# kei312/stereoanywhere

Hardware: AMD Instinct MI355X
Metric: stereo pairs/sec @540x960 D=192 (1/2/4/8 GPU) + EPE vs reference (higher is better)
Workload: dtype f32 (F(4x4) Winograd-domain and direct-conv products as exact f16 hi/lo pair products on MFMA, fp32 accumulation; everything else fp32); 1 GPU; configs[1]: batch 4/GPU x 540x960 (padded 544x960), 22 GRU iters, published flags; global_batch=4, iters=22, parallelism=dp1 (independent pairs, metrics all_gather)

## Files before the change

stereoanywhere_amd/csrc/conv2d_wino4.hip:

```cpp
#include "sa_common.h"

#include <algorithm>
#include <cstdlib>
#include <type_traits>

#pragma clang fp contract(fast)

namespace {

using sa::f32x4, sa::f32x2, sa::f16x2, sa::f16x4;

constexpr int NPT = 36;

template <int NW_, int KC_, bool SPLIT_ = false>
struct W4Cfg {
  static constexpr bool SPLIT = SPLIT_;
  static constexpr int NW = NW_, NTHR = 64 * NW_, TG = NW_ / 2, NT = 16 * TG, KC = KC_, JPC = KC_ / 4;
  static constexpr int NR = 6;
  static constexpr int CO = 32, CG = 2;
  static constexpr int SB = 4 * CO;
  static constexpr int PS_MAX = NT == 64 ? 340 : 204;
  static constexpr int PBUF = (KC * PS_MAX + 63) / 64 * 64 * 4;
  static constexpr int UBUF = NPT * KC * CO;
  static constexpr int BUF = PBUF + UBUF;
  static constexpr int OPP = NT * 16 + 4;
  static constexpr int SMEM = 2 * BUF > CO * OPP + CO * 9 + 8 ? 2 * BUF : CO * OPP + CO * 9 + 8;
  static constexpr int PDMA = ((KC * PS_MAX + 63) / 64 + NW - 1) / NW;
  static constexpr int UDMA = UBUF / 256;
  static constexpr int UPW = (UDMA + NW - 1) / NW;
  static_assert(SMEM * 4 <= 160 * 1024, "LDS budget");
  static constexpr int PPART = (PDMA > UPW ? PDMA : UPW) > 6 ? 3 : 2;
  static_assert(PDMA <= 3 * PPART && UPW <= 3 * PPART, "three DMA parts");
  static_assert(OPP % 32 == 4, "conflict-free staging");
  static constexpr int AFF_MAX = (160 * 1024 - SMEM * 4) / 8 > 512 ? 512 : (160 * 1024 - SMEM * 4) / 8;
};
using W4Big = W4Cfg<8, 8>;
using W4Small = W4Cfg<4, 4>;
using W4Split = W4Cfg<8, 8, true>;
constexpr int W4S_LOG2 = 12;
struct W4Half : W4Cfg<8, 8, true> {
  static constexpr bool HALF = true;
};
template <class C, class = void>
struct W4IsHalf : std::false_type {};
template <class C>
struct W4IsHalf<C, std::enable_if_t<C::HALF>> : std::true_type {};
static_assert(2 * W4Small::SMEM * 4 <= 160 * 1024, "two small blocks per CU");
template <class C, bool AFF>
constexpr bool W4Paired = C::SPLIT && C::JPC == 2 && !(W4IsHalf<C>::value && AFF);
constexpr int W4_GJB = 4;
constexpr int W4_GJB1 = 8;

struct W4Prob {
  const float *in;
  long in_bs;
  int Cin, H, W;
  const float *U;
  int Cout;
  const float *bias;
  int relu;
  float *out;
  long out_bs;
  int ltw;
  int tiles_w, tiles_hw, co_blocks;
  double *partial;
  const float *in_m, *in_s, *in_t;
  int in_pstride, in_act;
  int pitch;
  const float *skip;
  long skip_bs;
  const float *skip_s, *skip_t;
  int skip_act, out_act;
};
constexpr int MAX_PROB = 8;

__device__ __forceinline__ void w4_item(const unsigned wid, const int co_blocks, const int tiles_hw, int &cb, int &st,
                                        int &n) {
  cb = wid % co_blocks;
  const int gt = wid / co_blocks;
  st = gt % tiles_hw;
  n = gt / tiles_hw;
}
struct W4Gate {
  int mode;
  const float *ctx;
  long ctx_bs;
  const float *h;
  long h_bs;
  const float *z;
  long z_bs;
  const float *add;
  long add_bs;
  float *out2;
  long out2_bs;
  const float *head_w;
  float *head_part;
  long head_part_bs;
};
struct W4Launch {
  W4Prob p[MAX_PROB];
  W4Gate gate[MAX_PROB];
  unsigned end[MAX_PROB];
  unsigned nblk[MAX_PROB];
  int nprob;
  int guard;
};

__device__ __forceinline__ void w4_pair_split(const float x0, const float x1, f16x4 &ahi, f16x4 &alo) {
  const f16x2 h0 = __builtin_convertvector(f32x2{x0, x0}, f16x2);
  const f16x2 h1 = __builtin_convertvector(f32x2{x1, x1}, f16x2);
  float l0, l1;
  asm("v_fma_mix_f32 %0, -%1, 1.0, %2 op_sel_hi:[1,0,0]" : "=v"(l0) : "v"(__builtin_bit_cast(unsigned, h0)), "v"(x0));
  asm("v_fma_mix_f32 %0, -%1, 1.0, %2 op_sel_hi:[1,0,0]" : "=v"(l1) : "v"(__builtin_bit_cast(unsigned, h1)), "v"(x1));
  const f16x2 q0 = __builtin_convertvector(f32x2{l0, 0.0f}, f16x2);
  const f16x2 q1 = __builtin_convertvector(f32x2{l1, 0.0f}, f16x2);
  ahi = __builtin_shufflevector(h0, h1, 0, 1, 2, 3);
  alo = __builtin_shufflevector(q0, q1, 0, 1, 2, 3);
}

__device__ __forceinline__ f16x4 w4_pair_half(const float x0, const float x1) {
  const f16x2 h0 = __builtin_convertvector(f32x2{x0, x0}, f16x2);
  const f16x2 h1 = __builtin_convertvector(f32x2{x1, x1}, f16x2);
  return __builtin_shufflevector(h0, h1, 0, 1, 2, 3);
}

__device__ unsigned g_w4_redo_blocks;

__device__ __forceinline__ void dma16(__amdgpu_buffer_rsrc_t r, float *lds, int voff, int soff) {
  __builtin_amdgcn_raw_ptr_buffer_load_lds(r, (__attribute__((address_space(3))) void *)lds, 16, voff, soff, 0, 0);
}

__device__ __forceinline__ void bt6(const float x0, const float x1, const float x2, const float x3, const float x4,
                                    const float x5, float *o) {
  const float a = fmaf(-4.0f, x2, x4), b = fmaf(-4.0f, x1, x3), c = x4 - x2, e = x3 - x1;
  o[0] = fmaf(4.0f, x0, fmaf(-5.0f, x2, x4));
  o[1] = a + b;
  o[2] = a - b;
  o[3] = fmaf(2.0f, e, c);
  o[4] = fmaf(-2.0f, e, c);
  o[5] = fmaf(4.0f, x1, fmaf(-5.0f, x3, x5));
}

__device__ __forceinline__ void at6(const float *m, float *o) {
  const float a = m[1] + m[2], b = m[1] - m[2], c = m[3] + m[4], e = m[3] - m[4];
  o[0] = m[0] + a + c;
  o[1] = b + 2.0f * e;
  o[2] = a + 4.0f * c;
  o[3] = b + 8.0f * e + m[5];
}

template <int H>
__device__ __forceinline__ f32x4 at6h(const float u0, const float u1, const float u2) {
  if (H == 0) {
    const float p = u1 + u2, q = u1 - u2;
    return f32x4{u0 + p, q, p, q};
  } else {
    const float p = u0 + u1, q = u0 - u1;
    return f32x4{p, 2.0f * q, 4.0f * p, 8.0f * q + u2};
  }
}

__device__ __forceinline__ int w4_tile_of_row(int m) {
  const bool mid = m >= 4 && m < 12;
  const int j = mid ? m - 4 : (m < 4 ? m : m - 8);
  return (mid ? 0 : 2) + 4 * (j >> 1) + (j & 1);
}

template <int HF>
__device__ __forceinline__ void bt6h(const float x0, const float x1, const float x2, const float x3, const float x4,
                                     const float x5, float *o) {
  if (HF == 0) {
    const float a = fmaf(-4.0f, x2, x4), b = fmaf(-4.0f, x1, x3);
    o[0] = fmaf(4.0f, x0, fmaf(-5.0f, x2, x4));
    o[1] = a + b;
    o[2] = a - b;
  } else {
    const float c = x4 - x2, e = x3 - x1;
    o[0] = fmaf(2.0f, e, c);
    o[1] = fmaf(-2.0f, e, c);
    o[2] = fmaf(4.0f, x1, fmaf(-5.0f, x3, x5));
  }
}

template <class C, bool GATED, int NCH>
__device__ __forceinline__ void w4_emit(const W4Prob &P, const W4Gate *gate, const float *ot, const int cbase,
                                        const int n, const int co0, const int st, const int tiles_w, const int y0,
                                        const int x0, const int BH, const int BW, const int lbw, const int tid) {
  constexpr int NT = C::NT, NTHR = C::NTHR, OPP = C::OPP;
  const int H = P.H, W = P.W, Cout = P.Cout, pitch = P.pitch, hw = H * pitch;
  const int cb0 = co0 + cbase;
  auto tail0 = [&](f32x4 v, const int x) __attribute__((always_inline)) {
    if (x + 4 > W) {
#pragma unroll
      for (int e = 0; e < 4; ++e)
        if (x + e >= W) v[e] = 0.0f;
    }
    return v;
  };
  if (P.partial) {
    constexpr int NSUB = NT / 32, TPC = NTHR / (NCH * NSUB), PPT = 32 * 16 / TPC;
    const int c = tid / (TPC * NSUB), sub = (tid / TPC) % NSUB, part = tid % TPC;
    const int sub_rows = BH / NSUB, fine_h = (H + sub_rows - 1) / sub_rows;
    const int frow = (st / tiles_w) * NSUB + sub;
    double ssum = 0.0, ssq = 0.0;
#pragma unroll 2
    for (int p = sub * 512 + part * PPT; p < sub * 512 + (part + 1) * PPT; p += 4) {
      const int r = p >> lbw, cx = p & (BW - 1);
      if (y0 + r < H && x0 + cx < W) {
        const f32x4 v = tail0(*reinterpret_cast<const f32x4 *>(ot + c * OPP + p), x0 + cx);
#pragma unroll
        for (int e = 0; e < 4; ++e) {
          const double d = v[e];
          ssum += d;
          ssq += d * d;
        }
      }
    }
#pragma unroll
    for (int o = TPC / 2; o > 0; o >>= 1) {
      ssum += __shfl_xor(ssum, o);
      ssq += __shfl_xor(ssq, o);
    }
    if (part == 0 && frow < fine_h) {
      const long fst = (long)frow * tiles_w + st % tiles_w;
      double *pp = P.partial + (((long)n * Cout + cb0 + c) * ((long)fine_h * tiles_w) + fst) * 2;
      pp[0] = ssum;
      pp[1] = ssq;
    }
  }
  float *dst = P.out + (long)n * P.out_bs;
  constexpr int NJ = (NCH * NT * 16) / (4 * NTHR);
  auto plain_stores = [&]() __attribute__((always_inline)) {
    if (P.skip) {
      const float *sk = P.skip + (long)n * P.skip_bs;
#pragma unroll 4
      for (int j = 0; j < NJ; ++j) {
        const int i4 = tid + NTHR * j;
        const int c = i4 / (NT * 4), p = (i4 % (NT * 4)) * 4, r = p >> lbw, cx = p & (BW - 1);
        const int y = y0 + r, x = x0 + cx;
        if (y < H && x < W) {
          const long off = (long)(cb0 + c) * hw + (long)y * pitch + x;
          const f32x4 sv = *reinterpret_cast<const f32x4 *>(sk + off);
          const float ss = P.skip_s ? P.skip_s[cb0 + c] : 1.0f, st_ = P.skip_t ? P.skip_t[cb0 + c] : 0.0f;
          f32x4 v = *reinterpret_cast<const f32x4 *>(ot + c * OPP + p);
#pragma unroll
          for (int e = 0; e < 4; ++e) {
            float a = sv[e] * ss + st_;
            if (P.skip_act) a = fmaxf(a, 0.0f);
            v[e] = v[e] + a;
            if (P.out_act) v[e] = fmaxf(v[e], 0.0f);
          }
          *reinterpret_cast<f32x4 *>(dst + off) = tail0(v, x);
        }
      }
      return;
    }
#pragma unroll 4
    for (int j = 0; j < NJ; ++j) {
      const int i4 = tid + NTHR * j;
      const int c = i4 / (NT * 4), p = (i4 % (NT * 4)) * 4, r = p >> lbw, cx = p & (BW - 1);
      const int y = y0 + r, x = x0 + cx;
      if (y < H && x < W)
        *reinterpret_cast<f32x4 *>(dst + (long)(cb0 + c) * hw + (long)y * pitch + x) =
            tail0(*reinterpret_cast<const f32x4 *>(ot + c * OPP + p), x);
    }
  };
  if constexpr (!GATED) {
    plain_stores();
    return;
  } else {
  const W4Gate &GT = *gate;
  if (GT.mode == 0) {
    plain_stores();
    return;
  }
  const int half = Cout / 2;
// ... 123 lines not shown

template <class C, int LTW>
struct W4Geo {
  static constexpr int tw = 1 << LTW, tr = C::NT >> LTW;
  static constexpr int BH = 4 * tr, BW = 4 * tw, PG = tw + 2, PR = BH + 2, PS = PR * PG;
};

template <class C, bool AFF>
__device__ __forceinline__ float w4_guard_scale(const W4Prob &P, float *smem, const int n, const int nchunks,
                                                const int hw, const int (&po)[C::PDMA], const unsigned pcs,
                                                const int wv, const int lane) {
  constexpr int NWAVE = C::NW, KC = C::KC, PDMA = C::PDMA;
  float *red = smem;
  const char *ib = reinterpret_cast<const char *>(P.in + (long)n * P.in_bs);
  float mx = 0.0f;
#pragma unroll 8
  for (int kc = 0; kc < nchunks; ++kc)
#pragma unroll
    for (int j = 0; j < PDMA; ++j) {
      const int pcj = (int)((pcs >> (4 * j)) & 15u) - 1;
      if (pcj < 0) continue;
      const f32x4 v = *reinterpret_cast<const f32x4 *>(ib + po[j] + (long)kc * KC * hw * 4);
      float a = 1.0f, b = 0.0f, fl = -INFINITY;
      if constexpr (AFF) {
        const int pi = n * P.in_pstride + kc * KC + pcj;
        const float m0 = P.in_m ? P.in_m[pi] : 0.0f, t0 = P.in_t ? P.in_t[pi] : 0.0f;
        a = P.in_s ? P.in_s[pi] : 1.0f;
        b = t0 - m0 * a;
        fl = P.in_act ? 0.0f : -INFINITY;
      }
#pragma unroll
      for (int e = 0; e < 4; ++e) {
        const float t = __builtin_fabsf(fmaxf(v[e] * a + b, fl));
        mx = fmaxf(mx, t < INFINITY ? t : 0.0f);
      }
    }
  mx = sa::wave_max_dpp(mx);
  if (lane == 0) red[wv] = mx;
  __syncthreads();
  mx = red[0];
#pragma unroll
  for (int w = 1; w < NWAVE; ++w) mx = fmaxf(mx, red[w]);
  __syncthreads();
  int e2;
  (void)frexpf(100.0f * mx, &e2);
  return mx > 0.0f ? ldexpf(1.0f, 15 - e2) : 1.0f;
}

template <class C, int HF, int LTW, bool GATED, bool AFF>
__device__ __forceinline__ bool w4_body(const W4Prob &P, const W4Gate *gate, const unsigned wid, float *smem,
                                        float2 *atab, const bool guard = false, float xscale = 1.0f) {
  constexpr int NWAVE = C::NW, NTHR = C::NTHR, KC = C::KC, JPC = C::JPC, PDMA = C::PDMA,
                UDMA = C::UDMA, UPW = C::UPW, UBUF = C::UBUF, BUF = C::BUF, PBUF = C::PBUF, OPP = C::OPP,
                CO = C::CO, CG = C::CG, SB = C::SB, NR = C::NR;
  constexpr bool SPLIT = C::SPLIT, HALF = W4IsHalf<C>::value;
  static_assert(!SPLIT || NWAVE == 8, "split: the 8-wave shape");
  using f32xg = float __attribute__((ext_vector_type(CG)));
  const int Cin = P.Cin, H = P.H;
  using Geo = W4Geo<C, LTW>;
  constexpr int ltw = LTW, tw = Geo::tw, BH = Geo::BH, BW = Geo::BW, PG = Geo::PG, PS = Geo::PS;
  const int tid = threadIdx.x;
  const int lane = tid & 63;
  const int wv = __builtin_amdgcn_readfirstlane(tid >> 6);
  const int co_blocks = P.co_blocks, tiles_hw = P.tiles_hw, tiles_w = P.tiles_w;
  int cb, st, n;
  w4_item(wid, co_blocks, tiles_hw, cb, st, n);
  const int y0 = (st / tiles_w) * BH, x0 = (st % tiles_w) * BW;
  const int co0 = cb * CO;
  const int pitch = P.pitch, hw = H * pitch;
  const int nchunks = Cin / KC;

  const __amdgpu_buffer_rsrc_t xin = __builtin_amdgcn_make_buffer_rsrc(
      const_cast<float *>(P.in + (long)n * P.in_bs), (short)0, Cin * hw * 4, 0x00020000);
  const __amdgpu_buffer_rsrc_t uin = __builtin_amdgcn_make_buffer_rsrc(
      const_cast<float *>(P.U + (long)cb * Cin * NPT * CO), (short)0, Cin * NPT * CO * 4, 0x00020000);
  auto u_src = [&](int piece) {
    const int f = piece * 256 + lane * 4;
    return (JPC == 2 ? f : f + (f / SB) * SB) * 4;
  };
  auto u_chunk = [&](int chunk) {
    return JPC == 2 ? chunk * UBUF * 4 : (chunk >> 1) * 2 * UBUF * 4 + (chunk & 1) * SB * 4;
  };

#pragma unroll
  for (int j = 0; j < UPW; ++j)
    if (wv + NWAVE * j < UDMA)
      dma16(uin, smem + PBUF + (wv + NWAVE * j) * 256, u_src(wv + NWAVE * j), u_chunk(0));
  const int npi = (KC * PS + 63) >> 6;
  int po[PDMA];
  unsigned pcs = 0;
  static_assert(PDMA <= 8 && KC < 15, "4-bit channel fields");
#pragma unroll
  for (int j = 0; j < PDMA; ++j) {
    const int s = (wv + NWAVE * j) * 64 + lane;
    const int ci = s / PS, rem = s - ci * PS, r = rem / PG, g = rem - r * PG;
    const int y = y0 - 1 + r, x = x0 - 4 + 4 * g;
    const bool ok = s < KC * PS && y >= 0 && y < H && x >= 0 && x < pitch;
    po[j] = ok ? (ci * hw + y * pitch + x) * 4 : 0x7ffffff0;
    pcs |= (ok && wv + NWAVE * j < (KC * PS + 63) / 64 ? (unsigned)ci + 1u : 0u) << (4 * j);
  }
  if constexpr (SPLIT) {
    if (xscale == 0.0f) xscale = w4_guard_scale<C, AFF>(P, smem, n, nchunks, hw, po, pcs, wv, lane);
  }
  const bool scaled = xscale != 1.0f;
  auto issue_part = [&](int chunk, int buf, int part) __attribute__((always_inline)) {
    float *pb = smem + buf * BUF;
    const int xs = chunk * KC * hw * 4;
    float *ub = pb + PBUF;
    const int us = u_chunk(chunk);
#pragma unroll
    for (int j = 0; j < PDMA; ++j)
      if ((part < 0 || j / C::PPART == part) && wv + NWAVE * j < npi) dma16(xin, pb + (wv + NWAVE * j) * 256, po[j], xs);
#pragma unroll
    for (int j = 0; j < UPW; ++j)
      if ((part < 0 || j / C::PPART == part) && wv + NWAVE * j < UDMA)
        dma16(uin, ub + (wv + NWAVE * j) * 256, u_src(wv + NWAVE * j), us);
  };
  auto issue_p0 = [&]() __attribute__((always_inline)) {
#pragma unroll
    for (int j = 0; j < PDMA; ++j)
      if (wv + NWAVE * j < npi) dma16(xin, smem + (wv + NWAVE * j) * 256, po[j], 0);
  };

  const int tg = wv % C::TG;
  const int k = lane >> 4, m = lane & 15;
  const int tidx = tg * 16 + w4_tile_of_row(m), trow = tidx >> ltw, tcol = tidx & (tw - 1);
  int PSv = PS, PGv = PG;
  asm volatile("" : "+s"(PSv), "+s"(PGv));
  const int pread = k * PSv * 4 + 4 * trow * PGv * 4 + 4 * tcol + 2;
  const int uread = (k * 16 + m) * CG * (SPLIT ? JPC : 1);

  f32x4 acc[NR][3][CG];
#pragma unroll
  for (int i = 0; i < NR; ++i)
#pragma unroll
    for (int jj = 0; jj < 3; ++jj)
#pragma unroll
      for (int g = 0; g < CG; ++g) acc[i][jj][g] = f32x4{0.f, 0.f, 0.f, 0.f};

  float bpre[CG / 2];
#pragma unroll
  for (int k = 0; k < CG / 2; ++k) bpre[k] = P.bias ? P.bias[co0 + (2 * k + HF) * 16 + (lane & 15)] : 0.0f;
  if (HF == 1) __builtin_amdgcn_s_setprio(1);
  issue_p0();
  const float act_floor = P.in_act ? 0.0f : -INFINITY;
  if constexpr (AFF) {
    for (int c = tid; c < Cin; c += NTHR) {
      const int pi = n * P.in_pstride + c;
      const float m0 = P.in_m ? P.in_m[pi] : 0.0f, sc = P.in_s ? P.in_s[pi] : 1.0f, t0 = P.in_t ? P.in_t[pi] : 0.0f;
      atab[c] = make_float2(sc * xscale, (t0 - m0 * sc) * xscale);
    }
    __syncthreads();
  }
#pragma unroll 1
  for (int kc = 0; kc < nchunks; ++kc) {
    const int cur = kc & 1;
    if constexpr (AFF) {
      asm volatile("s_waitcnt vmcnt(0)" ::: "memory");
      float *pbuf = smem + cur * BUF;
#pragma unroll
      for (int j = 0; j < PDMA; ++j) {
        const int pcj = (int)((pcs >> (4 * j)) & 15u) - 1;
        if (pcj >= 0) {
          f32x4 *q = reinterpret_cast<f32x4 *>(pbuf + ((wv + NWAVE * j) * 64 + lane) * 4);
          const float2 ab = atab[kc * KC + pcj];
          f32x4 v = *q;
#pragma unroll
          for (int e = 0; e < 4; ++e) v[e] = fmaxf(v[e] * ab.x + ab.y, act_floor);
          *q = v;
        }
      }
    }
    if constexpr (SPLIT && !AFF) {
      if (scaled) {
        asm volatile("s_waitcnt vmcnt(0)" ::: "memory");
        float *pbuf = smem + cur * BUF + (wv * 64 + lane) * 4;
#pragma unroll 1
        for (int j = 0; j < PDMA; ++j) {
          if (wv + NWAVE * j < npi) {
            f32x4 *q = reinterpret_cast<f32x4 *>(pbuf + NWAVE * j * 256);
            *q = *q * xscale;
          }
        }
      }
    }
    __syncthreads();
    const float *pb = smem + cur * BUF + pread;
    const float *ub = smem + cur * BUF + PBUF + uread;
    f32x2 ra[6], rc[6];
    f32x4 rb[6];
    auto load_rows = [&](int s, int r0, int r1) __attribute__((always_inline)) {
      const float *p = pb + s * 4 * PSv * 4;
#pragma unroll
      for (int r = r0; r < r1; ++r) {
        ra[r] = *reinterpret_cast<const f32x2 *>(p + r * PGv * 4);
        rb[r] = *reinterpret_cast<const f32x4 *>(p + r * PGv * 4 + 2);
        rc[r] = *reinterpret_cast<const f32x2 *>(p + r * PGv * 4 + 6);
      }
    };
    f32xg bc[NR], bn[NR];
    auto load_b = [&](int s, int jj, f32xg *b) __attribute__((always_inline)) {
#pragma unroll
      for (int i = 0; i < NR; ++i) {
        if constexpr (SPLIT) {
          const float *q = ub + (6 * i + 3 * HF + jj) * JPC * SB + s;
          b[i] = f32xg{q[0], q[JPC]};
        } else {
          b[i] = *reinterpret_cast<const f32xg *>(ub + ((6 * i + 3 * HF + jj) * JPC + s) * SB);
        }
      }
    };
    if constexpr (W4Paired<C, AFF>) {
      float t0[6][3], t1[6][3];
      load_rows(0, 0, 6);
#pragma unroll
      for (int r = 0; r < 6; ++r) bt6h<HF>(ra[r].y, rb[r].x, rb[r].y, rb[r].z, rb[r].w, rc[r].x, t0[r]);
      load_rows(1, 0, 6);
#pragma unroll
      for (int r = 0; r < 6; ++r) bt6h<HF>(ra[r].y, rb[r].x, rb[r].y, rb[r].z, rb[r].w, rc[r].x, t1[r]);
      f32x4 pc_[NR];
      auto load_bp = [&](int jj, int i0, int i1, f32x4 (&b)[NR]) __attribute__((always_inline)) {
#pragma unroll
        for (int i = i0; i < i1; ++i) b[i] = *reinterpret_cast<const f32x4 *>(ub + (6 * i + 3 * HF + jj) * JPC * SB);
      };
#pragma unroll
      for (int jj = 0; jj < 3; ++jj) {
        if (kc + 1 < nchunks) {
          issue_part(kc + 1, cur ^ 1, jj);
          __builtin_amdgcn_sched_barrier(0);
        }
        load_bp(jj, 0, NR / 2, pc_);
        float v0[6], v1[6];
        bt6(t0[0][jj], t0[1][jj], t0[2][jj], t0[3][jj], t0[4][jj], t0[5][jj], v0);
        bt6(t1[0][jj], t1[1][jj], t1[2][jj], t1[3][jj], t1[4][jj], t1[5][jj], v1);
#pragma unroll
        for (int i = 0; i < NR; ++i) {
          if (i == 1) load_bp(jj, NR / 2, NR, pc_);
          if constexpr (HALF) {
            const f16x4 ahi = w4_pair_half(v0[i], v1[i]);
#pragma unroll
            for (int g = 0; g < CG; ++g) {
              const f16x4 bp = __builtin_bit_cast(f16x4, g == 0 ? pc_[i].xy : pc_[i].zw);
              acc[i][jj][g] = __builtin_amdgcn_mfma_f32_16x16x16f16(ahi, bp, acc[i][jj][g], 0, 0, 0);
            }
          } else {
            f16x4 ahi, alo;
            w4_pair_split(v0[i], v1[i], ahi, alo);
#pragma unroll
            for (int g = 0; g < CG; ++g) {
              const f16x4 bp = __builtin_bit_cast(f16x4, g == 0 ? pc_[i].xy : pc_[i].zw);
              acc[i][jj][g] = __builtin_amdgcn_mfma_f32_16x16x16f16(ahi, bp, acc[i][jj][g], 0, 0, 0);
              acc[i][jj][g] = __builtin_amdgcn_mfma_f32_16x16x16f16(alo, bp, acc[i][jj][g], 0, 0, 0);
            }
          }
        }
        __builtin_amdgcn_sched_barrier(0);
      }
    } else {
      load_rows(0, 0, 6);
      load_b(0, 0, bc);
#pragma unroll
      for (int s = 0; s < JPC; ++s) {
        if (s == 1) load_rows(1, 3, 6);
        float t[6][3];
#pragma unroll
        for (int r = 0; r < 6; ++r) bt6h<HF>(ra[r].y, rb[r].x, rb[r].y, rb[r].z, rb[r].w, rc[r].x, t[r]);
        if (s + 1 < JPC) load_rows(1, 0, 3);
#pragma unroll
        for (int jj = 0; jj < 3; ++jj) {
          if (s == 0 && kc + 1 < nchunks) {
            issue_part(kc + 1, cur ^ 1, jj);
            __builtin_amdgcn_sched_barrier(0);
          }
          if (s + 1 < JPC || jj < 2) load_b(jj < 2 ? s : s + 1, jj < 2 ? jj + 1 : 0, bn);
          float v[6];
          bt6(t[0][jj], t[1][jj], t[2][jj], t[3][jj], t[4][jj], t[5][jj], v);
          if constexpr (SPLIT) {
            static_assert(HALF, "an unpaired split config is the half config");
#pragma unroll
            for (int i = 0; i < NR; ++i) {
              const f16x4 a = __builtin_shufflevector(__builtin_convertvector(f32x2{v[i], v[i]}, f16x2),
                                                      f16x2{(_Float16)0.0f, (_Float16)0.0f}, 0, 1, 2, 3);
              const f16x4 b0 = __builtin_bit_cast(f16x4, f32x2{bc[i][0], bc[i][0]});
              const f16x4 b1 = __builtin_bit_cast(f16x4, f32x2{bc[i][1], bc[i][1]});
              acc[i][jj][0] = __builtin_amdgcn_mfma_f32_16x16x16f16(a, b0, acc[i][jj][0], 0, 0, 0);
              acc[i][jj][1] = __builtin_amdgcn_mfma_f32_16x16x16f16(a, b1, acc[i][jj][1], 0, 0, 0);
            }
          } else {
#pragma unroll
            for (int i = 0; i < NR; ++i)
#pragma unroll
              for (int g = 0; g < CG; ++g)
                acc[i][jj][g] = __builtin_amdgcn_mfma_f32_16x16x4f32(v[i], bc[i][g],
                                                                      acc[i][jj][g], 0, 0, 0);
          }
          __builtin_amdgcn_sched_barrier(0);

#pragma unroll
          for (int i = 0; i < NR; ++i) bc[i] = bn[i];
        }
      }
    }
  }
  __syncthreads();
  if constexpr (SPLIT) {
    const float inv_scale = 1.0f / ((float)(1 << W4S_LOG2) * xscale);
#pragma unroll
    for (int i = 0; i < NR; ++i)
#pragma unroll
      for (int jj = 0; jj < 3; ++jj)
#pragma unroll
        for (int g = 0; g < CG; ++g) acc[i][jj][g] *= inv_scale;
  }

  float *ot = smem;
  const int relu = P.relu;
  f32x4 chk = f32x4{0.f, 0.f, 0.f, 0.f};
  float whead = 0.0f;
  if constexpr (GATED && C::NTHR == 512)
    if (gate->mode == 3 && tid < C::CO * 9) whead = gate->head_w[co0 * 9 + tid];
#pragma unroll
  for (int phase = 0; phase < 2; ++phase) {
#pragma unroll
  for (int gi = 0; gi < CG / 2; ++gi) {
    const int g = 2 * gi + (phase == 0 ? 1 - HF : HF);
    const int col = g * 16 + (lane & 15);
    const float bv = phase == 1 ? bpre[gi] : 0.0f;
#pragma unroll
    for (int i = 0; i < 4; ++i) {
      const int ti = tg * 16 + w4_tile_of_row(4 * (lane >> 4) + i), orow = (ti >> ltw) * 4, ocol = (ti & (tw - 1)) * 4;
      float u[4][3];
#pragma unroll
      for (int jj = 0; jj < 3; ++jj) {
        float mcol[6], o[4];
#pragma unroll
        for (int a = 0; a < 6; ++a) mcol[a] = acc[a][jj][g][i];
        at6(mcol, o);
#pragma unroll
        for (int a = 0; a < 4; ++a) u[a][jj] = o[a];
      }
#pragma unroll
      for (int a = 0; a < 4; ++a) {
        const f32x4 y = at6h<HF>(u[a][0], u[a][1], u[a][2]);
        f32x4 *o = reinterpret_cast<f32x4 *>(ot + col * OPP + (orow + a) * BW + ocol);
        if (phase == 0) {
          *o = y;
        } else {
          f32x4 v = (HF == 0 ? (*o + y) : (y + *o)) + bv;
          if constexpr (SPLIT) chk += v;
          if (relu) v = f32x4{fmaxf(v.x, 0.0f), fmaxf(v.y, 0.0f), fmaxf(v.z, 0.0f), fmaxf(v.w, 0.0f)};
          *o = v;
        }
      }
    }
  }
    if (phase == 0) __syncthreads();
  }
  if constexpr (SPLIT) {
    static_assert(C::CO * C::OPP + C::CO * 9 + NWAVE <= C::SMEM, "range guard flags");
    int *flags = reinterpret_cast<int *>(smem + C::CO * C::OPP + C::CO * 9);
    const float t = (chk.x + chk.y) + (chk.z + chk.w);
    const bool wbad = __builtin_amdgcn_ballot_w64(!__builtin_isfinite(t)) != 0;
    if (lane == 0) flags[wv] = wbad ? 1 : 0;
    __syncthreads();
    int any = 0;
#pragma unroll
    for (int w = 0; w < NWAVE; ++w) any |= flags[w];
    if (any && guard) return true;
  } else {
    __syncthreads();
  }
  if constexpr (GATED && C::NTHR == 512) {
    if (gate->mode == 3) {
      w4_flowhead<C, LTW>(P, *gate, smem, n, co0, st, y0, x0, tid, whead);
      return false;
    }
  }
  w4_emit<C, GATED, C::CO>(P, gate, ot, 0, n, co0, st, tiles_w, y0, x0, BH, BW, ltw + 2, tid);
  return false;
}

template <class C, bool GATED, bool AFF = false>
__global__ __launch_bounds__(C::NTHR, C::NW == 8 ? 1 : 2) void wino_f4k3_kernel(const W4Launch L) {
  const unsigned g = blockIdx.x;
  int pi = 0;
#pragma unroll
  for (int i = 1; i < MAX_PROB; ++i) pi += (i < L.nprob && g >= L.end[i - 1]) ? 1 : 0;
  const unsigned base = pi ? L.end[pi - 1] : 0u, nb = L.nblk[pi];
  if (g - base >= nb) return;
  __shared__ __attribute__((aligned(16))) float smem[C::SMEM];
  __shared__ float2 atab[AFF ? C::AFF_MAX : 1];
  const unsigned wid = sa::xcd_remap(g - base, nb);
  const bool guard = C::SPLIT && L.guard;
  const W4Prob &P = L.p[pi];
  const W4Gate *gp = GATED ? &L.gate[pi] : nullptr;
  bool over;
#define W4_BODY(CC_, HF_, LTW_, G_, XS_) w4_body<CC_, HF_, LTW_, GATED, AFF>(P, gp, wid, smem, atab, G_, XS_)
  if (threadIdx.x < C::NTHR / 2) over = P.ltw == 4 ? W4_BODY(C, 0, 4, guard, 1.0f) : W4_BODY(C, 0, 5, guard, 1.0f);
  else over = P.ltw == 4 ? W4_BODY(C, 1, 4, guard, 1.0f) : W4_BODY(C, 1, 5, guard, 1.0f);
  if constexpr (C::SPLIT) {
    if (over) {
      __syncthreads();
      if (threadIdx.x == 0) atomicAdd(&g_w4_redo_blocks, 1u);
      int pil = __builtin_amdgcn_readfirstlane(pi);
      unsigned widl = __builtin_amdgcn_readfirstlane(wid);
      asm volatile("" : "+s"(pil), "+s"(widl));
      const W4Prob &P2 = L.p[pil];
      const W4Gate *gp2 = GATED ? &L.gate[pil] : nullptr;
#define W4_BODY2(HF_, LTW_) w4_body<C, HF_, LTW_, GATED, AFF>(P2, gp2, widl, smem, atab, false, 0.0f)
      if (threadIdx.x < C::NTHR / 2) {
        if (P2.ltw == 4) W4_BODY2(0, 4);
        else W4_BODY2(0, 5);
      } else {
        if (P2.ltw == 4) W4_BODY2(1, 4);
        else W4_BODY2(1, 5);
      }
#undef W4_BODY2
    }
  }
#undef W4_BODY
}

__global__ __launch_bounds__(256) void wino4_weights_kernel(const float *__restrict__ w, int Cout, int Cin, int CB,
                                                            float *__restrict__ U) {
  const long i = (long)blockIdx.x * blockDim.x + threadIdx.x;
  if (i >= (long)Cout * Cin) return;
  const int co = (int)(i / Cin), ci = (int)(i % Cin);
  const float *g = w + i * 9;
  const double G[6][3] = {{0.25, 0.0, 0.0},
                          {-1.0 / 6, -1.0 / 6, -1.0 / 6},
                          {-1.0 / 6, 1.0 / 6, -1.0 / 6},
                          {1.0 / 24, 1.0 / 12, 1.0 / 6},
                          {1.0 / 24, -1.0 / 12, 1.0 / 6},
                          {0.0, 0.0, 1.0}};
  double t[6][3];
  for (int a = 0; a < 6; ++a)
    for (int c = 0; c < 3; ++c) t[a][c] = G[a][0] * g[c] + G[a][1] * g[3 + c] + G[a][2] * g[6 + c];
  const int chunk = ci / 8, s = (ci % 8) / 4, k = ci % 4, cb = co / CB, c = co % CB, ng = CB / 16;
  for (int a = 0; a < 6; ++a)
    for (int b = 0; b < 6; ++b) {
      const double u = t[a][0] * G[b][0] + t[a][1] * G[b][1] + t[a][2] * G[b][2];
      const int pt = 6 * a + b;
      U[(((((long)cb * (Cin / 8) + chunk) * NPT + pt) * 2 + s) * 4 + k) * CB + (c & 15) * ng + (c >> 4)] = (float)u;
    }
}

__global__ __launch_bounds__(256) void wino4s_weights_kernel(const float *__restrict__ w, int Cout, int Cin,
                                                             unsigned *__restrict__ U) {
  const long i = (long)blockIdx.x * blockDim.x + threadIdx.x;
  if (i >= (long)Cout * Cin) return;
  const int co = (int)(i / Cin), ci = (int)(i % Cin);
  const float *g = w + i * 9;
  const double G[6][3] = {{0.25, 0.0, 0.0},
                          {-1.0 / 6, -1.0 / 6, -1.0 / 6},
                          {-1.0 / 6, 1.0 / 6, -1.0 / 6},
                          {1.0 / 24, 1.0 / 12, 1.0 / 6},
                          {1.0 / 24, -1.0 / 12, 1.0 / 6},
                          {0.0, 0.0, 1.0}};
  double t[6][3];
  for (int a = 0; a < 6; ++a)
    for (int c = 0; c < 3; ++c) t[a][c] = G[a][0] * g[c] + G[a][1] * g[3 + c] + G[a][2] * g[6 + c];
  const int chunk = ci / 8, s = (ci % 8) / 4, k = ci % 4, cb = co / 32, gg = (co % 32) / 16, n = co % 16;
  for (int a = 0; a < 6; ++a)
    for (int b = 0; b < 6; ++b) {
      const double u = (t[a][0] * G[b][0] + t[a][1] * G[b][1] + t[a][2] * G[b][2]) * (double)(1 << W4S_LOG2);
      const _Float16 hi = (_Float16)(float)u;
      const _Float16 lo = (_Float16)(float)(u - (double)hi);
      const unsigned pr = (unsigned)__builtin_bit_cast(unsigned short, hi) |
                          ((unsigned)__builtin_bit_cast(unsigned short, lo) << 16);
      const int pt = 6 * a + b;
      U[((((((long)cb * (Cin / 8) + chunk) * NPT + pt) * 4 + k) * 16 + n) * 2 + gg) * 2 + s] = pr;
    }
}


__global__ __launch_bounds__(256) void flow_head_reduce_kernel(const float *__restrict__ part, long part_bs, int ncb,
                                                               int H, int W, int BH, int BW, int tiles_w,
                                                               int tiles_hw, const float *__restrict__ bias0,
                                                               float *__restrict__ cx, float *__restrict__ fa,
                                                               long fa_bs, float *__restrict__ fb, long fb_bs) {
  const unsigned r = blockIdx.x * 256u + threadIdx.x;
  const unsigned hw = (unsigned)(H * W);
  if (r >= hw) return;
  const long b = blockIdx.y;
  const int y = (int)(r / (unsigned)W), x = (int)(r % (unsigned)W);
  const int RH = BH + 2, RW = BW + 2, tiles_h = tiles_hw / tiles_w;
  const int ty0 = y / BH, tx0 = x / BW;
  const bool up = y % BH == 0 && ty0 > 0, dn = y % BH == BH - 1 && ty0 + 1 < tiles_h;
  const bool lf = x % BW == 0 && tx0 > 0, rt = x % BW == BW - 1 && tx0 + 1 < tiles_w;
  const int ty1 = up ? ty0 - 1 : ty0 + 1, tx1 = lf ? tx0 - 1 : tx0 + 1;
  auto off = [&](int ty, int tx) { return ((long)(ty * tiles_w + tx) * RH + (y - (ty * BH - 1))) * RW + (x - (tx * BW - 1)); };
  const bool hy = up || dn, hx = lf || rt;
  const long o0 = off(ty0, tx0), o1 = hx ? off(ty0, tx1) : o0, o2 = hy ? off(ty1, tx0) : o0,
             o3 = hx && hy ? off(ty1, tx1) : o0;
  float d = bias0[0];
  const float *pc = part + b * part_bs;
  const long cbs = (long)tiles_hw * RH * RW;
  for (int cb0 = 0; cb0 < ncb; cb0 += 8) {
    float a[8][4];
#pragma unroll
    for (int j = 0; j < 8; ++j) {
      const float *q = pc + (long)min(cb0 + j, ncb - 1) * cbs;
      a[j][0] = q[o0];
      a[j][1] = q[o1];
      a[j][2] = q[o2];
      a[j][3] = q[o3];
    }
#pragma unroll
    for (int j = 0; j < 8; ++j) {
      const bool in = cb0 + j < ncb;
      d = in ? d + a[j][0] : d;
      d = in && hx ? d + a[j][1] : d;
      d = in && hy ? d + a[j][2] : d;
      d = in && hx && hy ? d + a[j][3] : d;
    }
  }
  const long i = b * hw + r;
  const float c = cx[i] + d;
  cx[i] = c;
  const float fx = c - (float)x;
  if (fa) {
    fa[b * fa_bs + r] = fx;
    fa[b * fa_bs + hw + r] = 0.0f;
  }
  if (fb) {
    fb[b * fb_bs + r] = fx;
    fb[b * fb_bs + hw + r] = 0.0f;
  }
}

int w4_ltw(int H, int W) {
  const long a16 = (long)((W + 63) / 64) * 64 * ((H + 15) / 16) * 16;
  const long a32 = (long)((W + 127) / 128) * 128 * ((H + 7) / 8) * 8;
  return a32 < a16 ? 5 : 4;
}

}

extern "C" int sa_conv2d_wino4_weights(const float *weight, int Cout, int Cin, float *U, void *stream) {
  SA_REQUIRE(weight && U && Cout > 0 && Cin > 0 && Cin % 8 == 0 && Cout % 32 == 0,
             "sa_conv2d_wino4_weights: bad arguments (Cin %% 8, Cout %% 32)");
  const long n = (long)Cout * Cin;
  hipStream_t s = sa::as_stream(stream);
  wino4_weights_kernel<<<(unsigned)((n + 255) / 256), 256, 0, s>>>(weight, Cout, Cin, 32, U);
  return sa::check_launch("sa_conv2d_wino4_weights");
}

extern "C" int sa_conv2d_wino4_weights_split(const float *weight, int Cout, int Cin, void *U, void *stream) {
  SA_REQUIRE(weight && U && Cout > 0 && Cin > 0 && Cin % 8 == 0 && Cout % 32 == 0,
             "sa_conv2d_wino4_weights_split: bad arguments (Cin %% 8, Cout %% 32)");
  const long n = (long)Cout * Cin;
  hipStream_t s = sa::as_stream(stream);
  wino4s_weights_kernel<<<(unsigned)((n + 255) / 256), 256, 0, s>>>(weight, Cout, Cin, static_cast<unsigned *>(U));
  return sa::check_launch("sa_conv2d_wino4_weights_split");
}

extern "C" long sa_flow_head_part_size(int N, int Cout, int H, int W) {
  if (N <= 0 || Cout <= 0 || Cout % 32 || H <= 0 || W <= 0) return -1;
  const int ltw = w4_ltw(H, W), bw = 4 << ltw, bh = 4 * (W4Big::NT >> ltw);
  const long tiles = (long)((W + bw - 1) / bw) * ((H + bh - 1) / bh);
  return (long)N * (Cout / 32) * tiles * (bh + 2) * (bw + 2);
}

extern "C" int sa_flow_head_reduce(const float *part, int N, int Cout, int H, int W, const float *bias0,
                                   float *coords_x, float *flow_a, long flow_a_bs, float *flow_b, long flow_b_bs,
                                   void *stream) {
  SA_REQUIRE(part && bias0 && coords_x, "sa_flow_head_reduce: null pointer");
  const long per = sa_flow_head_part_size(1, Cout, H, W);
  SA_REQUIRE(per > 0 && N > 0 && N <= 65535 && (long)H * W < (1L << 31), "sa_flow_head_reduce: bad shape");
  const int ltw = w4_ltw(H, W), bw = 4 << ltw, bh = 4 * (W4Big::NT >> ltw);
  const int tiles_w = (W + bw - 1) / bw, tiles_hw = tiles_w * ((H + bh - 1) / bh);
  const unsigned hw = (unsigned)((long)H * W);
  hipStream_t s = sa::as_stream(stream);
  sa::TimingScope ts(SA_K_PLUMBING, s);
  flow_head_reduce_kernel<<<dim3((hw + 255) / 256, N), 256, 0, s>>>(part, per, Cout / 32, H, W, bh, bw, tiles_w,
                                                                     tiles_hw, bias0, coords_x, flow_a, flow_a_bs,
                                                                     flow_b, flow_b_bs);
  return sa::check_launch("sa_flow_head_reduce");
}

long sa_direct_redo_blocks_internal(int reset);

extern "C" long sa_split_redo_blocks(int reset) {
  const long v = sa::read_redo_counter(g_w4_redo_blocks, reset);
  if (v < 0) return -1;
  const long d = sa_direct_redo_blocks_internal(reset);
  return d < 0 ? -1 : v + d;
}

extern "C" long sa_conv2d_k3_wino4_stat_parts(int H, int W) {
  const int ltw = w4_ltw(H, W), bw = 4 << ltw, bh = 4 * (32 >> ltw);
  return (long)((W + bw - 1) / bw) * ((H + bh - 1) / bh);
}

extern "C" int sa_conv2d_k3_wino4_multi(int nprob, const SaWinoProblem *probs, void *stream) {
  return sa_conv2d_k3_wino4_multi_gate(nprob, probs, nullptr, 0, stream);
}

extern "C" int sa_conv2d_k3_wino4_multi_gate(int nprob, const SaWinoProblem *probs, const SaGateEpilogue *gates,
                                             int block_shape, void *stream) {
  return sa_conv2d_k3_wino4_launch(nprob, probs, gates, block_shape, 0, stream);
}

extern "C" int sa_conv2d_k3_wino4_launch(int nprob, const SaWinoProblem *probs, const SaGateEpilogue *gates,
                                         int block_shape, int guard, void *stream) {
  SA_REQUIRE(nprob >= 1 && nprob <= MAX_PROB && probs, "sa_conv2d_k3_wino4_multi: 1..%d problems", MAX_PROB);
  SA_REQUIRE(block_shape == 0 || block_shape == 1 || block_shape == 2 || block_shape == 6 || block_shape == 7,
             "sa_conv2d_k3_wino4_multi: block_shape 0, 1, 2, 6 or 7 (got %d)", block_shape);
  const bool small = block_shape == 2, half = block_shape == 7, split = block_shape == 6 || half;
  const int nt = small ? W4Small::NT : W4Big::NT;
  constexpr int CO = 32;
  const int aff_max = small ? W4Small::AFF_MAX : split ? W4Split::AFF_MAX : W4Big::AFF_MAX;
  W4Launch L{};
  long total = 0;
  bool gated = false, aff = false;
  for (int i = 0; i < nprob; ++i) {
    const SaWinoProblem &q = probs[i];
    SA_REQUIRE(q.in && q.U && q.out && q.N > 0 && q.H > 0 && q.W > 0, "sa_conv2d_k3_wino4: bad arguments");
    SA_REQUIRE(q.Cin % 8 == 0 && q.Cout % CO == 0,
               "sa_conv2d_k3_wino4: needs Cin %% 8 == 0 and Cout %% 32 == 0 (got %d, %d)", q.Cin, q.Cout);
    const int pitch = q.pitch ? q.pitch : q.W;
    SA_REQUIRE(pitch >= q.W, "sa_conv2d_k3_wino4: pitch %d < W %d", pitch, q.W);
    SA_REQUIRE(pitch % 4 == 0 && (reinterpret_cast<uintptr_t>(q.in) & 15) == 0 && q.in_bs % 4 == 0 &&
                   (reinterpret_cast<uintptr_t>(q.out) & 15) == 0 && q.out_bs % 4 == 0 &&
                   (reinterpret_cast<uintptr_t>(q.U) & 15) == 0,
               "sa_conv2d_k3_wino4: needs W (or the row pitch) %% 4 == 0 and 16-byte aligned input / output planes "
               "and filters");
    const bool qaff = q.in_m || q.in_s || q.in_t || q.in_act;
    SA_REQUIRE(q.in_act == 0 || q.in_act == 1, "sa_conv2d_k3_wino4: input activation none or ReLU (got %d)", q.in_act);
    SA_REQUIRE(q.in_pstride == 0 || q.in_pstride == q.Cin, "sa_conv2d_k3_wino4: in_pstride must be 0 or Cin");
    SA_REQUIRE(!qaff || q.Cin <= aff_max, "sa_conv2d_k3_wino4: an input transform needs Cin <= %d", aff_max);
    aff = aff || qaff;
    SA_REQUIRE((long)q.Cin * q.H * pitch * 4 < (1L << 31) - 64 && 36L * q.Cin * q.Cout * 4 < (1L << 31),
               "sa_conv2d_k3_wino4: an image or the filter bank exceeds the 2 GB buffer-descriptor range");
    const int ltw = w4_ltw(q.H, q.W), bw = 4 << ltw, bh = 4 * (nt >> ltw);
    const int tiles_w = (q.W + bw - 1) / bw, tiles_h = (q.H + bh - 1) / bh;
    if (q.skip) {
      SA_REQUIRE(!q.stats_partial && !(gates && gates[i].mode != 0) && (reinterpret_cast<uintptr_t>(q.skip) & 15) == 0 &&
                     q.skip_bs % 4 == 0 && (q.skip_act == 0 || q.skip_act == 1) && (q.out_act == 0 || q.out_act == 1),
                 "sa_conv2d_k3_wino4: a residual epilogue takes no statistics or gate and a 16-byte aligned skip "
                 "plane (skip_act none or ReLU)");
    }
    L.p[i] = W4Prob{q.in, q.in_bs, q.Cin, q.H, q.W, q.U, q.Cout, q.bias, q.relu, q.out, q.out_bs,
                    ltw, tiles_w, tiles_w * tiles_h, q.Cout / CO, q.stats_partial,
                    q.in_m, q.in_s, q.in_t, q.in_pstride, q.in_act, pitch,
                    q.skip, q.skip_bs, q.skip_s, q.skip_t, q.skip_act, q.out_act};
    L.gate[i] = W4Gate{};
    if (gates && gates[i].mode != 0) {
      const SaGateEpilogue &e = gates[i];
      auto a16 = [](const void *p) { return (reinterpret_cast<uintptr_t>(p) & 15) == 0; };
      SA_REQUIRE(e.mode >= 1 && e.mode <= 3, "sa_conv2d_k3_wino4: gate mode %d", e.mode);
      if (e.mode == 3) {
        SA_REQUIRE(e.head_w && e.head_part && !q.stats_partial && !q.pitch && (block_shape == 0 || split),
                   "sa_conv2d_k3_wino4: the flow-head epilogue needs head_w / head_part, no statistics, dense "
                   "planes and the 8-wave 32-channel shape (block_shape 0, 6 or 7)");
        SA_REQUIRE(e.head_part_bs >= sa_flow_head_part_size(1, q.Cout, q.H, q.W),
                   "sa_conv2d_k3_wino4: head_part_bs too small");
        L.gate[i] = W4Gate{};
        L.gate[i].mode = 3;
        L.gate[i].head_w = e.head_w;
        L.gate[i].head_part = e.head_part;
        L.gate[i].head_part_bs = e.head_part_bs;
        gated = true;
        const long nb3 = (long)q.N * L.p[i].tiles_hw * L.p[i].co_blocks;
        total = (i + 1 < nprob ? (total + nb3 + 7) / 8 * 8 : total + nb3);
        SA_REQUIRE(total < (1L << 31), "sa_conv2d_k3_wino4: grid too large");
        L.end[i] = (unsigned)total;
        L.nblk[i] = (unsigned)nb3;
        continue;
      }
      SA_REQUIRE(!q.relu && !q.stats_partial, "sa_conv2d_k3_wino4: a gate epilogue takes no ReLU / statistics");
      SA_REQUIRE(e.ctx && e.h && a16(e.ctx) && a16(e.h) && e.ctx_bs % 4 == 0 && e.h_bs % 4 == 0,
                 "sa_conv2d_k3_wino4: gate needs 16-byte aligned ctx and h planes");
      if (e.mode == 1)
        SA_REQUIRE(q.Cout % (2 * CO) == 0 && e.out2 && a16(e.out2) && e.out2_bs % 4 == 0,
                   "sa_conv2d_k3_wino4: z/r gate needs Cout %% %d == 0 and an aligned r*h output", 2 * CO);
      else
        SA_REQUIRE(e.z && e.add && a16(e.z) && a16(e.add) && e.z_bs % 4 == 0 && e.add_bs % 4 == 0,
                   "sa_conv2d_k3_wino4: state gate needs aligned z and addend planes");
      L.gate[i] = W4Gate{e.mode, e.ctx, e.ctx_bs, e.h, e.h_bs, e.z, e.z_bs, e.add, e.add_bs, e.out2, e.out2_bs,
                         nullptr, nullptr, 0};
      gated = true;
    }
    const long nb = (long)q.N * L.p[i].tiles_hw * L.p[i].co_blocks;
    total = (i + 1 < nprob ? (total + nb + 7) / 8 * 8 : total + nb);
    SA_REQUIRE(total < (1L << 31), "sa_conv2d_k3_wino4: grid too large");
    L.end[i] = (unsigned)total;
    L.nblk[i] = (unsigned)nb;
  }
  for (int i = nprob; i < MAX_PROB; ++i) {
    L.end[i] = (unsigned)total;
    L.nblk[i] = 0;
  }
  L.nprob = nprob;
  SA_REQUIRE(!(aff && gated), "sa_conv2d_k3_wino4: an input transform and a gate epilogue in one launch");
  L.guard = split && guard ? 1 : 0;
  hipStream_t s = sa::as_stream(stream);
  sa::TimingScope ts(SA_K_CONV2D_W4, s);
  if (half) {
    aff     ? wino_f4k3_kernel<W4Half, false, true><<<(unsigned)total, W4Half::NTHR, 0, s>>>(L)
    : gated ? wino_f4k3_kernel<W4Half, true><<<(unsigned)total, W4Half::NTHR, 0, s>>>(L)
            : wino_f4k3_kernel<W4Half, false><<<(unsigned)total, W4Half::NTHR, 0, s>>>(L);
  } else if (split) {
    aff     ? wino_f4k3_kernel<W4Split, false, true><<<(unsigned)total, W4Split::NTHR, 0, s>>>(L)
    : gated ? wino_f4k3_kernel<W4Split, true><<<(unsigned)total, W4Split::NTHR, 0, s>>>(L)
            : wino_f4k3_kernel<W4Split, false><<<(unsigned)total, W4Split::NTHR, 0, s>>>(L);
// ... 14 lines not shown
```

Baseline: 68.88 pairs/s.

## Repack split Winograd weights for f32x4 loads and trim f16 pair conversions

Changes the split-weight layout so hi/lo halves sit in separate f16 slots. The unpaired split path can then load B operands as f32x4 with the same staged pattern as the paired path, instead of two scalar LDS reads per row. It also builds A operands from a single packed conversion using op_sel, and reuses a ring of persistent alo registers whose upper half stays zero so it is not rebuilt each time. The post-loop accumulator rescale is folded into the epilogue FMA with the bias. Together these cut LDS instructions, VALU conversions and epilogue multiplies, at the cost of subtle register-aliasing assumptions and a changed weight layout.

```diff
diff --git a/stereoanywhere_amd/csrc/conv2d_wino4.hip b/stereoanywhere_amd/csrc/conv2d_wino4.hip
--- a/stereoanywhere_amd/csrc/conv2d_wino4.hip
+++ b/stereoanywhere_amd/csrc/conv2d_wino4.hip
@@ -107,21 +107,28 @@
 };
 
 __device__ __forceinline__ void w4_pair_split(const float x0, const float x1, f16x4 &ahi, f16x4 &alo) {
-  const f16x2 h0 = __builtin_convertvector(f32x2{x0, x0}, f16x2);
-  const f16x2 h1 = __builtin_convertvector(f32x2{x1, x1}, f16x2);
+  const f16x2 p = __builtin_convertvector(f32x2{x0, x1}, f16x2);
+  const unsigned pu = __builtin_bit_cast(unsigned, p);
   float l0, l1;
-  asm("v_fma_mix_f32 %0, -%1, 1.0, %2 op_sel_hi:[1,0,0]" : "=v"(l0) : "v"(__builtin_bit_cast(unsigned, h0)), "v"(x0));
-  asm("v_fma_mix_f32 %0, -%1, 1.0, %2 op_sel_hi:[1,0,0]" : "=v"(l1) : "v"(__builtin_bit_cast(unsigned, h1)), "v"(x1));
-  const f16x2 q0 = __builtin_convertvector(f32x2{l0, 0.0f}, f16x2);
-  const f16x2 q1 = __builtin_convertvector(f32x2{l1, 0.0f}, f16x2);
-  ahi = __builtin_shufflevector(h0, h1, 0, 1, 2, 3);
-  alo = __builtin_shufflevector(q0, q1, 0, 1, 2, 3);
+  asm("v_fma_mix_f32 %0, -%1, 1.0, %2 op_sel_hi:[1,0,0]" : "=v"(l0) : "v"(pu), "v"(x0));
+  asm("v_fma_mix_f32 %0, -%1, 1.0, %2 op_sel:[1,0,0] op_sel_hi:[1,0,0]" : "=v"(l1) : "v"(pu), "v"(x1));
+  const f16x2 q = __builtin_convertvector(f32x2{l0, l1}, f16x2);
+  ahi = __builtin_shufflevector(p, p, 0, 1, 0, 1);
+  alo = __builtin_shufflevector(q, __builtin_shufflevector(alo, alo, 2, 3), 0, 1, 2, 3);
+}
+template <int N>
+__device__ __forceinline__ void w4_alo_init(f16x4 (&ring)[N]) {
+#pragma unroll
+  for (int r = 0; r < N; ++r) {
+    unsigned z = 0;
+    asm volatile("" : "+v"(z));
+    ring[r] = __builtin_bit_cast(f16x4, f32x2{__builtin_bit_cast(float, z), __builtin_bit_cast(float, z)});
+  }
 }
 
 __device__ __forceinline__ f16x4 w4_pair_half(const float x0, const float x1) {
-  const f16x2 h0 = __builtin_convertvector(f32x2{x0, x0}, f16x2);
-  const f16x2 h1 = __builtin_convertvector(f32x2{x1, x1}, f16x2);
-  return __builtin_shufflevector(h0, h1, 0, 1, 2, 3);
+  const f16x2 p = __builtin_convertvector(f32x2{x0, x1}, f16x2);
+  return __builtin_shufflevector(p, p, 0, 1, 0, 1);
 }
 
 __device__ unsigned g_w4_redo_blocks;
@@ -551,6 +558,9 @@
     }
     __syncthreads();
   }
+  constexpr int W4_ALO = AFF ? 1 : 2;
+  f16x4 alo_ring[W4_ALO];
+  if constexpr (W4Paired<C, AFF> && !HALF) w4_alo_init(alo_ring);
 #pragma unroll 1
   for (int kc = 0; kc < nchunks; ++kc) {
     const int cur = kc & 1;
@@ -600,14 +610,12 @@
     f32xg bc[NR], bn[NR];
     auto load_b = [&](int s, int jj, f32xg *b) __attribute__((always_inline)) {
 #pragma unroll
-      for (int i = 0; i < NR; ++i) {
-        if constexpr (SPLIT) {
-          const float *q = ub + (6 * i + 3 * HF + jj) * JPC * SB + s;
-          b[i] = f32xg{q[0], q[JPC]};
-        } else {
-          b[i] = *reinterpret_cast<const f32xg *>(ub + ((6 * i + 3 * HF + jj) * JPC + s) * SB);
-        }
-      }
+      for (int i = 0; i < NR; ++i) b[i] = *reinterpret_cast<const f32xg *>(ub + ((6 * i + 3 * HF + jj) * JPC + s) * SB);
+    };
+    f32x4 pc_[NR];
+    auto load_bp = [&](int jj, int i0, int i1) __attribute__((always_inline)) {
+#pragma unroll
+      for (int i = i0; i < i1; ++i) pc_[i] = *reinterpret_cast<const f32x4 *>(ub + (6 * i + 3 * HF + jj) * JPC * SB);
     };
     if constexpr (W4Paired<C, AFF>) {
       float t0[6][3], t1[6][3];
@@ -617,24 +625,19 @@
       load_rows(1, 0, 6);
 #pragma unroll
       for (int r = 0; r < 6; ++r) bt6h<HF>(ra[r].y, rb[r].x, rb[r].y, rb[r].z, rb[r].w, rc[r].x, t1[r]);
-      f32x4 pc_[NR];
-      auto load_bp = [&](int jj, int i0, int i1, f32x4 (&b)[NR]) __attribute__((always_inline)) {
-#pragma unroll
-        for (int i = i0; i < i1; ++i) b[i] = *reinterpret_cast<const f32x4 *>(ub + (6 * i + 3 * HF + jj) * JPC * SB);
-      };
 #pragma unroll
       for (int jj = 0; jj < 3; ++jj) {
         if (kc + 1 < nchunks) {
           issue_part(kc + 1, cur ^ 1, jj);
           __builtin_amdgcn_sched_barrier(0);
         }
-        load_bp(jj, 0, NR / 2, pc_);
+        load_bp(jj, 0, NR / 2);
         float v0[6], v1[6];
         bt6(t0[0][jj], t0[1][jj], t0[2][jj], t0[3][jj], t0[4][jj], t0[5][jj], v0);
         bt6(t1[0][jj], t1[1][jj], t1[2][jj], t1[3][jj], t1[4][jj], t1[5][jj], v1);
 #pragma unroll
         for (int i = 0; i < NR; ++i) {
-          if (i == 1) load_bp(jj, NR / 2, NR, pc_);
+          if (i == 1) load_bp(jj, NR / 2, NR);
           if constexpr (HALF) {
             const f16x4 ahi = w4_pair_half(v0[i], v1[i]);
 #pragma unroll
@@ -643,7 +646,9 @@
               acc[i][jj][g] = __builtin_amdgcn_mfma_f32_16x16x16f16(ahi, bp, acc[i][jj][g], 0, 0, 0);
             }
           } else {
-            f16x4 ahi, alo;
+            f16x4 ahi;
+            f16x4 &alo = alo_ring[(NR * jj + i) % W4_ALO];
+            static_assert(3 * NR % W4_ALO == 0, "the rotation closes over a chunk");
             w4_pair_split(v0[i], v1[i], ahi, alo);
 #pragma unroll
             for (int g = 0; g < CG; ++g) {
@@ -657,7 +662,7 @@
       }
     } else {
       load_rows(0, 0, 6);
-      load_b(0, 0, bc);
+      if constexpr (!SPLIT) load_b(0, 0, bc);
 #pragma unroll
       for (int s = 0; s < JPC; ++s) {
         if (s == 1) load_rows(1, 3, 6);
@@ -671,17 +676,20 @@
             issue_part(kc + 1, cur ^ 1, jj);
             __builtin_amdgcn_sched_barrier(0);
           }
-          if (s + 1 < JPC || jj < 2) load_b(jj < 2 ? s : s + 1, jj < 2 ? jj + 1 : 0, bn);
+          if constexpr (SPLIT) load_bp(jj, 0, NR / 2);
+          else if (s + 1 < JPC || jj < 2) load_b(jj < 2 ? s : s + 1, jj < 2 ? jj + 1 : 0, bn);
           float v[6];
           bt6(t[0][jj], t[1][jj], t[2][jj], t[3][jj], t[4][jj], t[5][jj], v);
           if constexpr (SPLIT) {
             static_assert(HALF, "an unpaired split config is the half config");
 #pragma unroll
             for (int i = 0; i < NR; ++i) {
-              const f16x4 a = __builtin_shufflevector(__builtin_convertvector(f32x2{v[i], v[i]}, f16x2),
-                                                      f16x2{(_Float16)0.0f, (_Float16)0.0f}, 0, 1, 2, 3);
-              const f16x4 b0 = __builtin_bit_cast(f16x4, f32x2{bc[i][0], bc[i][0]});
-              const f16x4 b1 = __builtin_bit_cast(f16x4, f32x2{bc[i][1], bc[i][1]});
+              if (i == 1) load_bp(jj, NR / 2, NR);
+              const f16x2 h = __builtin_convertvector(s == 0 ? f32x2{v[i], 0.0f} : f32x2{0.0f, v[i]}, f16x2);
+              const f16x4 a = __builtin_shufflevector(h, h, 0, 1, 0, 1);
+              const f32x2 g0 = pc_[i].xy, g1 = pc_[i].zw;
+              const f16x4 b0 = __builtin_bit_cast(f16x4, g0);
+              const f16x4 b1 = __builtin_bit_cast(f16x4, g1);
               acc[i][jj][0] = __builtin_amdgcn_mfma_f32_16x16x16f16(a, b0, acc[i][jj][0], 0, 0, 0);
               acc[i][jj][1] = __builtin_amdgcn_mfma_f32_16x16x16f16(a, b1, acc[i][jj][1], 0, 0, 0);
             }
@@ -695,22 +703,16 @@
           }
           __builtin_amdgcn_sched_barrier(0);
 
-#pragma unroll
-          for (int i = 0; i < NR; ++i) bc[i] = bn[i];
+          if constexpr (!SPLIT) {
+#pragma unroll
+            for (int i = 0; i < NR; ++i) bc[i] = bn[i];
+          }
         }
       }
     }
   }
   __syncthreads();
-  if constexpr (SPLIT) {
-    const float inv_scale = 1.0f / ((float)(1 << W4S_LOG2) * xscale);
-#pragma unroll
-    for (int i = 0; i < NR; ++i)
-#pragma unroll
-      for (int jj = 0; jj < 3; ++jj)
-#pragma unroll
-        for (int g = 0; g < CG; ++g) acc[i][jj][g] *= inv_scale;
-  }
+  const float inv_scale = SPLIT ? 1.0f / ((float)(1 << W4S_LOG2) * xscale) : 1.0f;
 
   float *ot = smem;
   const int relu = P.relu;
@@ -745,8 +747,14 @@
         if (phase == 0) {
           *o = y;
         } else {
-          f32x4 v = (HF == 0 ? (*o + y) : (y + *o)) + bv;
-          if constexpr (SPLIT) chk += v;
+          f32x4 v = HF == 0 ? (*o + y) : (y + *o);
+          if constexpr (SPLIT) {
+            v = f32x4{fmaf(v.x, inv_scale, bv), fmaf(v.y, inv_scale, bv), fmaf(v.z, inv_scale, bv),
+                      fmaf(v.w, inv_scale, bv)};
+            chk += v;
+          } else {
+            v = v + bv;
+          }
           if (relu) v = f32x4{fmaxf(v.x, 0.0f), fmaxf(v.y, 0.0f), fmaxf(v.z, 0.0f), fmaxf(v.w, 0.0f)};
           *o = v;
         }
@@ -845,7 +853,7 @@
 }
 
 __global__ __launch_bounds__(256) void wino4s_weights_kernel(const float *__restrict__ w, int Cout, int Cin,
-                                                             unsigned *__restrict__ U) {
+                                                             unsigned short *__restrict__ U) {
   const long i = (long)blockIdx.x * blockDim.x + threadIdx.x;
   if (i >= (long)Cout * Cin) return;
   const int co = (int)(i / Cin), ci = (int)(i % Cin);
@@ -865,10 +873,10 @@
       const double u = (t[a][0] * G[b][0] + t[a][1] * G[b][1] + t[a][2] * G[b][2]) * (double)(1 << W4S_LOG2);
       const _Float16 hi = (_Float16)(float)u;
       const _Float16 lo = (_Float16)(float)(u - (double)hi);
-      const unsigned pr = (unsigned)__builtin_bit_cast(unsigned short, hi) |
-                          ((unsigned)__builtin_bit_cast(unsigned short, lo) << 16);
       const int pt = 6 * a + b;
-      U[((((((long)cb * (Cin / 8) + chunk) * NPT + pt) * 4 + k) * 16 + n) * 2 + gg) * 2 + s] = pr;
+      unsigned short *q = U + (((((((long)cb * (Cin / 8) + chunk) * NPT + pt) * 4 + k) * 16 + n) * 2 + gg) * 4 + s);
+      q[0] = __builtin_bit_cast(unsigned short, hi);
+      q[2] = __builtin_bit_cast(unsigned short, lo);
     }
 }
 
@@ -950,7 +958,7 @@
              "sa_conv2d_wino4_weights_split: bad arguments (Cin %% 8, Cout %% 32)");
   const long n = (long)Cout * Cin;
   hipStream_t s = sa::as_stream(stream);
-  wino4s_weights_kernel<<<(unsigned)((n + 255) / 256), 256, 0, s>>>(weight, Cout, Cin, static_cast<unsigned *>(U));
+  wino4s_weights_kernel<<<(unsigned)((n + 255) / 256), 256, 0, s>>>(weight, Cout, Cin, static_cast<unsigned short *>(U));
   return sa::check_launch("sa_conv2d_wino4_weights_split");
 }
 
```

After: 69.82 pairs/s, median of 6. 1.4% higher.
